# yml-bit/CTA-GAN

Measured on AMD Instinct MI355X. Metric: paired 512x512 slices/sec (G+D step); generator rel-L2 vs CPU reference, higher is better.
Workload: dtype bf16; 1 GPU; HdGan stage-2 full G+D train step (G, Reg, STN, D_m, losses, Adam x3), 16 paired 512x512 slices/GPU; per_gpu_batch=16, global_batch=16, size=512, parallelism=single, rccl_ranks=1, dp_backend=none

## Files before the change

### cta_gan_amd/csrc/common.h

```cpp
#pragma once
#include <hip/hip_runtime.h>
#include <stdint.h>
#include <utility>
#include "../../include/ctagan_hip.h"

#define CTG_OK 0
#define CTG_EINVAL 1

enum { DT_F32 = 0, DT_BF16 = 1, DT_PAIR = 2, DT_MIX = 3 };
enum { ACT_NONE = 0, ACT_RELU = 1, ACT_LRELU = 2, ACT_TANH = 3, ACT_SIGMOID = 4 };
enum { PAD_ZERO = 0, PAD_REFLECT = 1 };

typedef __bf16 bf16_t;
struct bfpair_t { bf16_t v; };
typedef float f32x4 __attribute__((ext_vector_type(4)));
typedef unsigned u32x4 __attribute__((ext_vector_type(4)));
typedef __bf16 bf16x8 __attribute__((ext_vector_type(8)));
typedef __bf16 bf16x4 __attribute__((ext_vector_type(4)));

#define LRELU_SLOPE 0.2f

#define CTG_ENTER() (void)hipGetLastError()

static inline int ctg_launch_status() {
// ... 72 lines not shown
template <> struct Chunk<bfpair_t> {
    static constexpr int N = 8;
    float v[8];
    struct Raw { u32x4 h, l; };
    static __device__ __forceinline__ Raw fetch(const bfpair_t* p, int ld) {
        return Raw{*reinterpret_cast<const u32x4*>(p), *reinterpret_cast<const u32x4*>(p + (ld >> 1))};
    }
    __device__ __forceinline__ void unpack(const Raw& t) {
#pragma unroll
        for (int i = 0; i < 4; ++i) {
            v[2 * i] = __uint_as_float(t.h[i] << 16) + __uint_as_float(t.l[i] << 16);
            v[2 * i + 1] = __uint_as_float(t.h[i] & 0xffff0000u) + __uint_as_float(t.l[i] & 0xffff0000u);
        }
    }
    __device__ __forceinline__ void load(const bfpair_t* p, int ld) { unpack(fetch(p, ld)); }
    __device__ __forceinline__ void store(bfpair_t* p, int ld) const {
        bf16x8 h, l;
#pragma unroll
        for (int i = 0; i < 8; ++i) {
            h[i] = (bf16_t)v[i];
            l[i] = (bf16_t)(v[i] - (float)h[i]);
        }
        *reinterpret_cast<bf16x8*>(p) = h;
        *reinterpret_cast<bf16x8*>(p + (ld >> 1)) = l;
    }
    __device__ __forceinline__ void zero() {
#pragma unroll
        for (int i = 0; i < 8; ++i) v[i] = 0.f;
    }
};
template <typename T> struct PlanesOf { static constexpr int N = 1; };
template <> struct PlanesOf<bfpair_t> { static constexpr int N = 2; };

__device__ __forceinline__ float ld1(const float* p) { return *p; }
__device__ __forceinline__ float ld1(const bf16_t* p) { return (float)*p; }
__device__ __forceinline__ void st1(float* p, float v) { *p = v; }
__device__ __forceinline__ void st1(bf16_t* p, float v) { *p = (bf16_t)v; }

__device__ __forceinline__ float act_apply(float x, int act) {
    switch (act) {
        case ACT_RELU: return x > 0.f ? x : 0.f;
        case ACT_LRELU: return x > 0.f ? x : LRELU_SLOPE * x;
        case ACT_TANH: return tanhf(x);
        case ACT_SIGMOID: return 1.f / (1.f + __expf(-x));
        default: return x;
    }
}
__device__ __forceinline__ float act_grad_from_out(float y, int act) {
    switch (act) {
        case ACT_RELU: return y > 0.f ? 1.f : 0.f;
        case ACT_LRELU: return y > 0.f ? 1.f : LRELU_SLOPE;
        case ACT_TANH: return 1.f - y * y;
        case ACT_SIGMOID: return y * (1.f - y);
        default: return 1.f;
    }
}

template <typename F, int... I>
__device__ __forceinline__ void static_for_impl(F&& f, std::integer_sequence<int, I...>) {
    (f(std::integral_constant<int, I>{}), ...);
}
template <int N, typename F> __device__ __forceinline__ void static_for(F&& f) {
    static_for_impl(static_cast<F&&>(f), std::make_integer_sequence<int, N>{});
}

#define IN_EPS 1e-5f
// ... 36 lines not shown
```

### cta_gan_amd/csrc/conv_wgrad.hip

```cpp
#include <stdlib.h>
#include "conv_dispatch.h"

struct WgradArgs {
    const void* g;
    const void* x;
    float* part;
    int B, Hs, Ws, Mc, g_ld;
    int Hi, Wi, Nc, x_ld;
    int is, pad_mode;
    int slab, sps;
    int ntaps;
    int taps[64];
};

template <typename T> struct WgCfg;
template <> struct WgCfg<bf16_t> { static constexpr int PK = 64, PK_MT = 32, PADB = 32; };
template <> struct WgCfg<float> { static constexpr int PK = 32, PK_MT = 16, PADB = 64; };

template <typename T, int BM, int BN, int NT>
__global__ __launch_bounds__(256) void conv_wgrad_kernel(const WgradArgs a) {
    constexpr int EPC = VecOf<T>::N;
    constexpr int PK = NT > 1 ? WgCfg<T>::PK_MT : WgCfg<T>::PK;
    constexpr int RSM = BM * (int)sizeof(T) + WgCfg<T>::PADB;
    constexpr int RSN = BN * (int)sizeof(T) + WgCfg<T>::PADB;
// ... 919 lines not shown
            const int bm = h.Mc % 64 == 0 ? 64 : h.Mc % 32 == 0 ? 32 : 16, bn = h.Nc % 64 == 0 ? 64 : 32;
            ok = ok && bm >= 32 && !(bm == 32 && bn == 32) && (cnt == 1 || cnt == 2 || cnt == 4) && kw <= 2 && kh <= 2;
            covered += cnt;
            ++nph;
        }
        if (ok && covered == ntaps && ntaps == 9 && nph == 4 && !split) {
            if (taps_3x3(a.taps, false)) {
                WgHaloArgs h = ph[0];
                h.ntaps = 9; h.gtaps = 9; h.kw = 2; h.khb = 2; h.dy0 = -1; h.dx0 = -1; h.py = 0; h.px = 0;
                const int rc = launch_wg_s2m(h, st);
                if (rc != -1) return rc;
            }
        }
        if (ok && covered == ntaps) {
            for (int p = 0; p < nph; ++p) {
                const int rc = launch_wgh_any(ph[p], st);
                if (rc != 0) return rc == -1 ? CTG_EINVAL : rc;
            }
            return split ? 3 : 0;
        }
    }
    if (pair) return 2;
    if (Mc % 32) return CTG_EINVAL;
    return dtype == DT_BF16 ? launch_wg_t<bf16_t>(a, st) : launch_wg_t<float>(a, st);
}

#define RED_MAX_T 24
struct ReduceList {
    const float* part[RED_MAX_T];
    float* dst[RED_MAX_T];
    long sm[RED_MAX_T], sn[RED_MAX_T], stp[RED_MAX_T];
    int Z[RED_MAX_T], ntaps[RED_MAX_T], Mc[RED_MAX_T], Nc[RED_MAX_T], Mreal[RED_MAX_T], Nreal[RED_MAX_T];
    int acc[RED_MAX_T], shift[RED_MAX_T];
    int first[RED_MAX_T + 1];
    int count;
};

__global__ __launch_bounds__(256) void wgrad_reduce_multi_kernel(const ReduceList L) {
    __shared__ float red[256];
    int j = 0;
    while (j + 1 < L.count && (int)blockIdx.x >= L.first[j + 1]) ++j;
    const int shift = L.shift[j], ZP = 1 << shift, IW = 256 >> shift;
    const int il = threadIdx.x & (IW - 1), zq = threadIdx.x >> (8 - shift);
    const int Z = L.Z[j], Mc = L.Mc[j], Nc = L.Nc[j];
    const long E = (long)L.ntaps[j] * Mc * Nc;
    const long idx = (long)((int)blockIdx.x - L.first[j]) * IW + il;
    const float* __restrict__ part = L.part[j];
    float s0 = 0.f, s1 = 0.f, s2 = 0.f, s3 = 0.f;
    if (idx < E) {
        int zz = zq;
        for (; zz + 3 * ZP < Z; zz += 4 * ZP) {
            s0 += part[(long)zz * E + idx];
            s1 += part[(long)(zz + ZP) * E + idx];
            s2 += part[(long)(zz + 2 * ZP) * E + idx];
            s3 += part[(long)(zz + 3 * ZP) * E + idx];
        }
        for (; zz < Z; zz += ZP) s0 += part[(long)zz * E + idx];
    }
    float s = (s0 + s1) + (s2 + s3);
    if (shift) {
        red[zq * IW + il] = s;
        __syncthreads();
        s = 0.f;
        if (zq == 0)
            for (int q = 0; q < ZP; ++q) s += red[q * IW + il];
    }
    if (zq == 0 && idx < E) {
        const int c = (int)(idx % Nc);
        const int m = (int)((idx / Nc) % Mc);
        const int t = (int)(idx / ((long)Nc * Mc));
        if (m < L.Mreal[j] && c < L.Nreal[j]) {
            float* d = L.dst[j] + m * L.sm[j] + c * L.sn[j] + t * L.stp[j];
            *d = L.acc[j] ? *d + s : s;
        }
    }
}

extern "C" int ctg_wgrad_reduce_multi(int count, const void* const* part, void* const* dst, const int* Z,
                                      const int* ntaps, const int* Mc, const int* Nc, const int* Mreal, const int* Nreal,
                                      const long* sm, const long* sn, const long* stp, const int* accumulate,
                                      void* stream) {
    CTG_ENTER();
    if (count < 0) return CTG_EINVAL;
    for (int base = 0; base < count; base += RED_MAX_T) {
        ReduceList L;
        L.count = count - base < RED_MAX_T ? count - base : RED_MAX_T;
        long blocks = 0;
        for (int i = 0; i < L.count; ++i) {
            const int q = base + i;
            if (Z[q] < 1 || ntaps[q] < 1 || Mreal[q] > Mc[q] || Nreal[q] > Nc[q] || part[q] == nullptr || dst[q] == nullptr)
                return CTG_EINVAL;
            const long E = (long)ntaps[q] * Mc[q] * Nc[q];
            const int shift = (Z[q] >= 64 && E <= 65536) ? (E <= 16384 ? 5 : 4) : 0;
            L.part[i] = (const float*)part[q]; L.dst[i] = (float*)dst[q];
            L.sm[i] = sm[q]; L.sn[i] = sn[q]; L.stp[i] = stp[q];
            L.Z[i] = Z[q]; L.ntaps[i] = ntaps[q]; L.Mc[i] = Mc[q]; L.Nc[i] = Nc[q]; L.Mreal[i] = Mreal[q]; L.Nreal[i] = Nreal[q];
            L.acc[i] = accumulate[q]; L.shift[i] = shift;
            L.first[i] = (int)blocks;
            const int iw = 256 >> shift;
            blocks += (E + iw - 1) / iw;
            if (blocks >= (1L << 30)) return CTG_EINVAL;
        }
        L.first[L.count] = (int)blocks;
        if (blocks == 0) continue;
        hipLaunchKernelGGL(wgrad_reduce_multi_kernel, dim3((unsigned)blocks), dim3(256), 0, (hipStream_t)stream, L);
    }
    return ctg_launch_status();
}

extern "C" int ctg_wgrad_reduce(const float* part, int Z, int ntaps, int Mc, int Nc, float* dst, int Mreal, int Nreal,
                                long sm, long sn, long stp, int accumulate, void* stream) {
    CTG_ENTER();
    if (Z < 1 || ntaps < 1 || Mreal > Mc || Nreal > Nc) return CTG_EINVAL;
    const long E = (long)ntaps * Mc * Nc;
    if (Z >= 64 && E <= 65536) {
        if (E <= 16384) {
            hipLaunchKernelGGL(wgrad_reduce_zp_kernel<32>, dim3((unsigned)((E + 7) / 8)), dim3(256), 0,
                               (hipStream_t)stream, part, Z, ntaps, Mc, Nc, dst, Mreal, Nreal, sm, sn, stp, accumulate);
        } else {
            hipLaunchKernelGGL(wgrad_reduce_zp_kernel<16>, dim3((unsigned)((E + 15) / 16)), dim3(256), 0,
                               (hipStream_t)stream, part, Z, ntaps, Mc, Nc, dst, Mreal, Nreal, sm, sn, stp, accumulate);
        }
        return ctg_launch_status();
    }
    const int blocks = (int)((E + 255) / 256 < 4096 ? (E + 255) / 256 : 4096);
    hipLaunchKernelGGL(wgrad_reduce_kernel, dim3(blocks), dim3(256), 0, (hipStream_t)stream, part, Z, ntaps, Mc, Nc,
                       dst, Mreal, Nreal, sm, sn, stp, accumulate);
    return ctg_launch_status();
}
```

### cta_gan_amd/csrc/spatial.hip

```cpp
#include "common.h"

static inline int ew_blocks(long items) {
    long b = (items + 255) / 256;
    return (int)(b < 1 ? 1 : (b > 8192 ? 8192 : b));
}

#define DISPATCH_T(dtype, CALL)                   \
    if ((dtype) == DT_BF16) { typedef bf16_t T; CALL; } \
    else if ((dtype) == DT_F32) { typedef float T; CALL; } \
    else if ((dtype) == DT_PAIR) { typedef bfpair_t T; CALL; } \
    else return CTG_EINVAL;

template <typename T>
__global__ void maxpool2_fwd_kernel(const T* __restrict__ x, int x_ld, T* __restrict__ out, int o_ld, int H, int W,
                                    int C, long items) {
    constexpr int EPC = Chunk<T>::N;
    const int CPP = C / EPC, Ho = H / 2, Wo = W / 2;
    for (long it = (long)blockIdx.x * blockDim.x + threadIdx.x; it < items; it += (long)gridDim.x * blockDim.x) {
        const unsigned pixu = (unsigned)it / (unsigned)CPP;
        const long pix = pixu;
        const int ch = (int)(it - pix * CPP) * EPC;
        const int ox = (int)(pixu % (unsigned)Wo);
        const int oy = (int)((pixu / (unsigned)Wo) % (unsigned)Ho);
        const int n = (int)(pixu / ((unsigned)Wo * (unsigned)Ho));
        const T* base = x + (((size_t)n * H + 2 * oy) * W + 2 * ox) * x_ld + ch;
        Chunk<T> a, b, c, d, o;
        a.load(base, x_ld); b.load(base + x_ld, x_ld); c.load(base + (size_t)W * x_ld, x_ld); d.load(base + (size_t)(W + 1) * x_ld, x_ld);
#pragma unroll
        for (int e = 0; e < EPC; ++e) o.v[e] = fmaxf(fmaxf(a.v[e], b.v[e]), fmaxf(c.v[e], d.v[e]));
        o.store(out + pix * o_ld + ch, o_ld);
    }
}

template <typename T, typename TX = T>
__global__ void maxpool2_bwd_kernel(const TX* __restrict__ x, int x_ld, const T* __restrict__ dout, int d_ld,
                                    T* __restrict__ dx, int dx_ld, int accumulate, int H, int W, int C, long items) {
    constexpr int EPC = Chunk<T>::N;
    const int CPP = C / EPC, Ho = H / 2, Wo = W / 2;
    for (long it = (long)blockIdx.x * blockDim.x + threadIdx.x; it < items; it += (long)gridDim.x * blockDim.x) {
        const unsigned pixu = (unsigned)it / (unsigned)CPP;
        const long pix = pixu;
        const int ch = (int)(it - pix * CPP) * EPC;
        const int xx = (int)(pixu % (unsigned)W);
        const int y = (int)((pixu / (unsigned)W) % (unsigned)H);
        const int n = (int)(pixu / ((unsigned)W * (unsigned)H));
        const int oy = y >> 1, ox = xx >> 1;
        Chunk<T> o;
        o.zero();
        if (oy < Ho && ox < Wo) {
            const TX* base = x + (((size_t)n * H + 2 * oy) * W + 2 * ox) * x_ld + ch;
            Chunk<TX> w[4];
            Chunk<T> g;
            w[0].load(base, x_ld); w[1].load(base + x_ld, x_ld); w[2].load(base + (size_t)W * x_ld, x_ld);
            w[3].load(base + (size_t)(W + 1) * x_ld, x_ld);
            g.load(dout + (((size_t)n * Ho + oy) * Wo + ox) * d_ld + ch, d_ld);
            const int me = (y & 1) * 2 + (xx & 1);
#pragma unroll
            for (int e = 0; e < EPC; ++e) {
                int arg = 0;
                float m = w[0].v[e];
#pragma unroll
                for (int k = 1; k < 4; ++k)
                    if (w[k].v[e] > m) { m = w[k].v[e]; arg = k; }
                o.v[e] = arg == me ? g.v[e] : 0.f;
            }
        }
        T* dst = dx + pix * dx_ld + ch;
        if (accumulate) {
            Chunk<T> prev;
            prev.load(dst, dx_ld);
#pragma unroll
            for (int e = 0; e < EPC; ++e) o.v[e] += prev.v[e];
        }
        o.store(dst, dx_ld);
    }
}

__device__ __forceinline__ void bil_src(int o, float scale, int Hi, int& i0, int& i1, float& l) {
    float s = scale * ((float)o + 0.5f) - 0.5f;
    s = s < 0.f ? 0.f : s;
    i0 = (int)s;
    i1 = i0 + (i0 < Hi - 1 ? 1 : 0);
    l = s - (float)i0;
}

template <typename T>
__global__ void bilinear_fwd_kernel(const T* __restrict__ x, int x_ld, T* __restrict__ out, int o_ld, int Hi, int Wi,
                                    int Ho, int Wo, int C, long items) {
    constexpr int EPC = Chunk<T>::N;
    const int CPP = C / EPC;
    const float sh = (float)Hi / (float)Ho, sw = (float)Wi / (float)Wo;
    for (long it = (long)blockIdx.x * blockDim.x + threadIdx.x; it < items; it += (long)gridDim.x * blockDim.x) {
        const unsigned pixu = (unsigned)it / (unsigned)CPP;
        const long pix = pixu;
        const int ch = (int)(it - pix * CPP) * EPC;
        const int ox = (int)(pixu % (unsigned)Wo);
        const int oy = (int)((pixu / (unsigned)Wo) % (unsigned)Ho);
        const int n = (int)(pixu / ((unsigned)Wo * (unsigned)Ho));
        int y0, y1, x0, x1;
        float ly, lx;
        bil_src(oy, sh, Hi, y0, y1, ly);
        bil_src(ox, sw, Wi, x0, x1, lx);
        const T* b = x + (size_t)n * Hi * Wi * x_ld + ch;
        Chunk<T> v00, v01, v10, v11, o;
        v00.load(b + ((size_t)y0 * Wi + x0) * x_ld, x_ld); v01.load(b + ((size_t)y0 * Wi + x1) * x_ld, x_ld);
        v10.load(b + ((size_t)y1 * Wi + x0) * x_ld, x_ld); v11.load(b + ((size_t)y1 * Wi + x1) * x_ld, x_ld);
        const float hy = 1.f - ly, hx = 1.f - lx;
#pragma unroll
        for (int e = 0; e < EPC; ++e)
            o.v[e] = hy * (hx * v00.v[e] + lx * v01.v[e]) + ly * (hx * v10.v[e] + lx * v11.v[e]);
        o.store(out + pix * o_ld + ch, o_ld);
    }
}

template <typename T>
__global__ void bilinear_bwd_kernel(const T* __restrict__ dout, int d_ld, T* __restrict__ dx, int dx_ld, int Hi,
                                    int Wi, int Ho, int Wo, int C, long items) {
    constexpr int EPC = Chunk<T>::N;
    const int CPP = C / EPC;
    const float sh = (float)Hi / (float)Ho, sw = (float)Wi / (float)Wo;
    for (long it = (long)blockIdx.x * blockDim.x + threadIdx.x; it < items; it += (long)gridDim.x * blockDim.x) {
        const unsigned pixu = (unsigned)it / (unsigned)CPP;
        const long pix = pixu;
        const int ch = (int)(it - pix * CPP) * EPC;
        const int ix = (int)(pixu % (unsigned)Wi);
        const int iy = (int)((pixu / (unsigned)Wi) % (unsigned)Hi);
        const int n = (int)(pixu / ((unsigned)Wi * (unsigned)Hi));
        float wy[5], wx[5];
#pragma unroll
        for (int k = 0; k < 5; ++k) {
            const int oy = 2 * iy - 2 + k, ox = 2 * ix - 2 + k;
            wy[k] = 0.f; wx[k] = 0.f;
            if (oy >= 0 && oy < Ho) {
                int a0, a1; float l;
                bil_src(oy, sh, Hi, a0, a1, l);
                wy[k] = (a0 == iy ? 1.f - l : 0.f) + (a1 == iy ? l : 0.f);
            }
            if (ox >= 0 && ox < Wo) {
                int a0, a1; float l;
                bil_src(ox, sw, Wi, a0, a1, l);
                wx[k] = (a0 == ix ? 1.f - l : 0.f) + (a1 == ix ? l : 0.f);
            }
        }
        Chunk<T> o;
        o.zero();
        const T* b = dout + (size_t)n * Ho * Wo * d_ld + ch;
        for (int a = 0; a < 5; ++a) {
            if (wy[a] == 0.f) continue;
            const int oy = 2 * iy - 2 + a;
            for (int c = 0; c < 5; ++c) {
                if (wx[c] == 0.f) continue;
                const int ox = 2 * ix - 2 + c;
                Chunk<T> g;
                g.load(b + ((size_t)oy * Wo + ox) * d_ld, d_ld);
                const float w = wy[a] * wx[c];
#pragma unroll
                for (int e = 0; e < EPC; ++e) o.v[e] += w * g.v[e];
            }
        }
        o.store(dx + pix * dx_ld + ch, dx_ld);
    }
}

template <typename T>
__global__ void chan_pad_kernel(const float* __restrict__ src, int Cs, T* __restrict__ dst, int Cpad, long P) {
    constexpr int EPC = Chunk<T>::N;
    const int CPP = Cpad / EPC;
    for (long pix = (long)blockIdx.x * blockDim.x + threadIdx.x; pix < P; pix += (long)gridDim.x * blockDim.x) {
        Chunk<T> o;
        o.zero();
        if (Cs == 2 && ((uintptr_t)src & 7) == 0) {
            const float2 v = *reinterpret_cast<const float2*>(src + pix * 2);
            o.v[0] = v.x; o.v[1] = v.y;
        } else {
            for (int c = 0; c < Cs; ++c) o.v[c] = src[pix * Cs + c];
        }
        constexpr int PL = PlanesOf<T>::N;
        T* d = dst + pix * Cpad * PL;
        o.store(d, Cpad * PL);
        o.zero();
        for (int cc = 1; cc < CPP; ++cc) o.store(d + cc * EPC, Cpad * PL);
    }
}

template <typename T>
__global__ void im2col_pack_kernel(const float* __restrict__ s0, const float* __restrict__ s1, int Cin, int Hi, int Wi,
                                   int kh, int kw, int stride, int pad, int pad_mode, T* __restrict__ dst, int Ho,
                                   int Wo, int Kpad, long items) {
    constexpr int EPC = Chunk<T>::N;
    const int CPP = Kpad / EPC;
    const int K = Cin * kh * kw;
    for (long it = (long)blockIdx.x * blockDim.x + threadIdx.x; it < items; it += (long)gridDim.x * blockDim.x) {
        const unsigned pixu = (unsigned)it / (unsigned)CPP;
        const long pix = pixu;
        const int cc = (int)(it - pix * CPP);
        const int ox = (int)(pixu % (unsigned)Wo);
        const int oy = (int)((pixu / (unsigned)Wo) % (unsigned)Ho);
        const int n = (int)(pixu / ((unsigned)Wo * (unsigned)Ho));
        Chunk<T> o;
#pragma unroll
        for (int e = 0; e < EPC; ++e) {
            const int k = cc * EPC + e;
            float v = 0.f;
            if (k < K) {
                const int c = k / (kh * kw);
                const int r = k - c * kh * kw;
                const int ky = r / kw, kx = r - ky * kw;
                int iy = oy * stride - pad + ky, ix = ox * stride - pad + kx;
                bool ok = true;
                if (pad_mode == PAD_REFLECT) { iy = reflect_idx(iy, Hi); ix = reflect_idx(ix, Wi); }
                else ok = (unsigned)iy < (unsigned)Hi && (unsigned)ix < (unsigned)Wi;
                if (ok) v = (c == 0 ? s0 : s1)[((size_t)n * Hi + iy) * Wi + ix];
            }
            o.v[e] = v;
        }
        o.store(dst + pix * Kpad * PlanesOf<T>::N + cc * EPC, Kpad * PlanesOf<T>::N);
    }
}

template <typename T>
__global__ void copy_channels_kernel(const T* __restrict__ src, int s_ld, T* __restrict__ dst, int d_ld, int C,
                                     long items) {
    constexpr int EPC = Chunk<T>::N;
    const int CPP = C / EPC;
    for (long it = (long)blockIdx.x * blockDim.x + threadIdx.x; it < items; it += (long)gridDim.x * blockDim.x) {
        const unsigned pixu = (unsigned)it / (unsigned)CPP;
        const long pix = pixu;
        const int ch = (int)(it - pix * CPP) * EPC;
        *reinterpret_cast<u32x4*>(dst + pix * d_ld + ch) = *reinterpret_cast<const u32x4*>(src + pix * s_ld + ch);
        if constexpr (PlanesOf<T>::N == 2)
            *reinterpret_cast<u32x4*>(dst + pix * d_ld + (d_ld >> 1) + ch) = *reinterpret_cast<const u32x4*>(src + pix * s_ld + (s_ld >> 1) + ch);
    }
}

extern "C" int ctg_maxpool2_fwd(int dtype, const void* x, int x_ld, void* out, int o_ld, int B, int H, int W, int C,
                                void* stream) {
    CTG_ENTER();
    const int epc = dtype == DT_F32 ? 4 : 8;
    if (C % epc || H < 2 || W < 2) return CTG_EINVAL;
    const long items = (long)B * (H / 2) * (W / 2) * (C / epc);
    if (items >= (1L << 31)) return CTG_EINVAL;
    DISPATCH_T(dtype, hipLaunchKernelGGL((maxpool2_fwd_kernel<T>), dim3(ew_blocks(items)), dim3(256), 0,
                                         (hipStream_t)stream, (const T*)x, x_ld, (T*)out, o_ld, H, W, C, items));
    return ctg_launch_status();
}

extern "C" int ctg_maxpool2_bwd(int dtype, const void* x, int x_ld, const void* dout, int d_ld, void* dx, int dx_ld,
                                int accumulate, int B, int H, int W, int C, void* stream) {
    CTG_ENTER();
    const int epc = dtype == DT_F32 ? 4 : 8;
    if (C % epc || H < 2 || W < 2) return CTG_EINVAL;
    const long items = (long)B * H * W * (C / epc);
    if (items >= (1L << 31)) return CTG_EINVAL;
    if (dtype == DT_MIX) {
        hipLaunchKernelGGL((maxpool2_bwd_kernel<bf16_t, bfpair_t>), dim3(ew_blocks(items)), dim3(256), 0, (hipStream_t)stream,
                           (const bfpair_t*)x, x_ld, (const bf16_t*)dout, d_ld, (bf16_t*)dx, dx_ld, accumulate, H, W, C, items);
        return ctg_launch_status();
    }
    DISPATCH_T(dtype, hipLaunchKernelGGL((maxpool2_bwd_kernel<T>), dim3(ew_blocks(items)), dim3(256), 0,
                                         (hipStream_t)stream, (const T*)x, x_ld, (const T*)dout, d_ld, (T*)dx, dx_ld,
                                         accumulate, H, W, C, items));
    return ctg_launch_status();
}

extern "C" int ctg_bilinear_fwd(int dtype, const void* x, int x_ld, void* out, int o_ld, int B, int Hi, int Wi, int Ho,
                                int Wo, int C, void* stream) {
    CTG_ENTER();
    const int epc = dtype == DT_F32 ? 4 : 8;
    if (C % epc) return CTG_EINVAL;
    const long items = (long)B * Ho * Wo * (C / epc);
    if (items >= (1L << 31)) return CTG_EINVAL;
    DISPATCH_T(dtype, hipLaunchKernelGGL((bilinear_fwd_kernel<T>), dim3(ew_blocks(items)), dim3(256), 0,
                                         (hipStream_t)stream, (const T*)x, x_ld, (T*)out, o_ld, Hi, Wi, Ho, Wo, C,
                                         items));
    return ctg_launch_status();
}

extern "C" int ctg_bilinear_bwd(int dtype, const void* dout, int d_ld, void* dx, int dx_ld, int B, int Hi, int Wi,
                                int Ho, int Wo, int C, void* stream) {
    CTG_ENTER();
    const int epc = dtype == DT_F32 ? 4 : 8;
    if (C % epc || Ho != 2 * Hi || Wo != 2 * Wi) return CTG_EINVAL;
    const long items = (long)B * Hi * Wi * (C / epc);
    if (items >= (1L << 31)) return CTG_EINVAL;
    DISPATCH_T(dtype, hipLaunchKernelGGL((bilinear_bwd_kernel<T>), dim3(ew_blocks(items)), dim3(256), 0,
                                         (hipStream_t)stream, (const T*)dout, d_ld, (T*)dx, dx_ld, Hi, Wi, Ho, Wo, C,
                                         items));
    return ctg_launch_status();
}

__global__ void split_weights_kernel(const float* __restrict__ x, long x_ld, bf16_t* __restrict__ out, int C, long P) {
    const int cpp = C / 8;
    const long items = P * cpp;
    for (long it = (long)blockIdx.x * blockDim.x + threadIdx.x; it < items; it += (long)gridDim.x * blockDim.x) {
        const long p = it / cpp;
        const int c = (int)(it - p * cpp) * 8;
        const float* src = x + p * x_ld + c;
        const f32x4 a = *reinterpret_cast<const f32x4*>(src), b = *reinterpret_cast<const f32x4*>(src + 4);
        bf16x8 hi, lo;
#pragma unroll
        for (int e = 0; e < 4; ++e) {
            hi[e] = (bf16_t)a[e];
            lo[e] = (bf16_t)(a[e] - (float)hi[e]);
            hi[4 + e] = (bf16_t)b[e];
            lo[4 + e] = (bf16_t)(b[e] - (float)hi[4 + e]);
        }
        bf16_t* row = out + p * (2L * C);
        const int j = c >> 5, i = c & 31;
        *reinterpret_cast<bf16x8*>(row + 64 * j + i) = hi;
        *reinterpret_cast<bf16x8*>(row + 64 * j + 32 + i) = lo;
    }
}

extern "C" int ctg_split_weights(const float* x, long x_ld, void* out, int C, long P, void* stream) {
    CTG_ENTER();
    if (C < 32 || C % 32 || x_ld < C || x_ld % 4 || P < 1 || ((uintptr_t)x & 15) || ((uintptr_t)out & 15)) return CTG_EINVAL;
    hipLaunchKernelGGL(split_weights_kernel, dim3(ew_blocks(P * (C / 8))), dim3(256), 0, (hipStream_t)stream, x, x_ld,
                       (bf16_t*)out, C, P);
    return ctg_launch_status();
}
// ... 75 lines not shown
    const int cpp = C / 8;
    for (long it = (long)blockIdx.x * blockDim.x + threadIdx.x; it < items; it += (long)gridDim.x * blockDim.x) {
        const long p = it / cpp;
        const int c = (int)(it - p * cpp) * 8;
        Chunk<bfpair_t> v;
        v.load(src + p * s_ld + c, s_ld);
        Chunk<float> a, b;
#pragma unroll
        for (int e = 0; e < 4; ++e) { a.v[e] = v.v[e]; b.v[e] = v.v[4 + e]; }
        a.store(dst + p * d_ld + c);
        b.store(dst + p * d_ld + c + 4);
    }
}

extern "C" int ctg_pair_convert(int dir, const void* src, long s_ld, void* dst, long d_ld, int C, long P, void* stream) {
    CTG_ENTER();
    if (C < 8 || C % 8 || P < 1 || (dir != 0 && dir != 1) || ((uintptr_t)src & 15) || ((uintptr_t)dst & 15)) return CTG_EINVAL;
    const long pl = dir == 0 ? d_ld : s_ld, fl = dir == 0 ? s_ld : d_ld;
    if (pl < 2 * C || pl % 16 || pl >= (1L << 31) || fl < C || fl % 4) return CTG_EINVAL;
    const long items = P * (C / 8);
    if (dir == 0)
        hipLaunchKernelGGL(pair_from_f32_kernel, dim3(ew_blocks(items)), dim3(256), 0, (hipStream_t)stream, (const float*)src,
                           s_ld, (bfpair_t*)dst, (int)d_ld, C, items);
    else
        hipLaunchKernelGGL(pair_to_f32_kernel, dim3(ew_blocks(items)), dim3(256), 0, (hipStream_t)stream,
                           (const bfpair_t*)src, (int)s_ld, (float*)dst, d_ld, C, items);
    return ctg_launch_status();
}

extern "C" int ctg_chan_pad(int dtype, const float* src, int Cs, void* dst, int Cpad, long P, void* stream) {
    CTG_ENTER();
    const int epc = dtype == DT_F32 ? 4 : 8;
    if (Cs < 1 || Cs > 4 || Cpad % epc || P * (Cpad / epc) >= (1L << 31)) return CTG_EINVAL;
    DISPATCH_T(dtype, hipLaunchKernelGGL((chan_pad_kernel<T>), dim3(ew_blocks(P)), dim3(256), 0,
                                         (hipStream_t)stream, src, Cs, (T*)dst, Cpad, P));
    return ctg_launch_status();
}

extern "C" int ctg_im2col_pack(int dtype, const float* s0, const float* s1, int Cin, int B, int Hi, int Wi, int kh,
                               int kw, int stride, int pad, int pad_mode, void* dst, int Ho, int Wo, int Kpad,
                               void* stream) {
    CTG_ENTER();
    const int epc = dtype == DT_F32 ? 4 : 8;
    if (Cin < 1 || Cin > 2 || (Cin == 2 && s1 == nullptr) || Kpad % epc || Kpad < Cin * kh * kw) return CTG_EINVAL;
    if (pad_mode == PAD_REFLECT && (pad >= Hi || pad >= Wi)) return CTG_EINVAL;
    if (Ho != (Hi + 2 * pad - kh) / stride + 1 || Wo != (Wi + 2 * pad - kw) / stride + 1) return CTG_EINVAL;
    const long items = (long)B * Ho * Wo * (Kpad / epc);
    if (items >= (1L << 31)) return CTG_EINVAL;
    DISPATCH_T(dtype, hipLaunchKernelGGL((im2col_pack_kernel<T>), dim3(ew_blocks(items)), dim3(256), 0,
                                         (hipStream_t)stream, s0, s1, Cin, Hi, Wi, kh, kw, stride, pad, pad_mode,
                                         (T*)dst, Ho, Wo, Kpad, items));
    return ctg_launch_status();
}

extern "C" int ctg_copy_channels(int dtype, const void* src, int s_ld, void* dst, int d_ld, int C, long P,
                                 void* stream) {
    CTG_ENTER();
    const int epc = dtype == DT_F32 ? 4 : 8;
    if (C % epc || s_ld % epc || d_ld % epc) return CTG_EINVAL;
    const long items = P * (C / epc);
    if (items >= (1L << 31)) return CTG_EINVAL;
    DISPATCH_T(dtype, hipLaunchKernelGGL((copy_channels_kernel<T>), dim3(ew_blocks(items)), dim3(256), 0,
                                         (hipStream_t)stream, (const T*)src, s_ld, (T*)dst, d_ld, C, items));
    return ctg_launch_status();
}

extern "C" int ctg_abi_version(void) { return CTG_ABI_VERSION; }
```

Baseline: 332.5 slices/s.

## Restructure spatial elementwise kernels around per-output-cell streaming and vectorized wgrad reduce

Maxpool backward now runs one thread per pooled cell that writes all four input pixels, instead of one thread per input pixel that re-reads the whole 2x2 window. Bilinear 2x upsampling forward and backward get dedicated kernels that share neighbour loads across output pixels, driven by a generic issue/finish item-streaming helper. Channel padding is parallelised per chunk rather than per pixel, and the wgrad split-K reduction gains a float4-vectorised path with deeper load batching. These changes aim to cut redundant global loads and index arithmetic in memory-bound kernels, at the cost of more code and per-item register pressure.

```diff
diff --git a/cta_gan_amd/csrc/common.h b/cta_gan_amd/csrc/common.h
--- a/cta_gan_amd/csrc/common.h
+++ b/cta_gan_amd/csrc/common.h
@@ -128,6 +128,65 @@
 template <typename T> struct PlanesOf { static constexpr int N = 1; };
 template <> struct PlanesOf<bfpair_t> { static constexpr int N = 2; };
 
+struct ItemPos { int c, x, y, n; };
+__device__ __forceinline__ ItemPos item_decode(unsigned it, int CPP, int W, int H) {
+    ItemPos p;
+    const unsigned pix = it / (unsigned)CPP, row = pix / (unsigned)W;
+    p.c = (int)(it - pix * (unsigned)CPP);
+    p.x = (int)(pix - row * (unsigned)W);
+    p.n = (int)(row / (unsigned)H);
+    p.y = (int)(row - (unsigned)p.n * (unsigned)H);
+    return p;
+}
+__device__ __forceinline__ void item_advance(ItemPos& p, const ItemPos& d, int CPP, int W, int H) {
+    p.c += d.c;
+    int k = p.c >= CPP ? 1 : 0;
+    p.c -= k ? CPP : 0;
+    p.x += d.x + k;
+    k = p.x >= W ? 1 : 0;
+    p.x -= k ? W : 0;
+    p.y += d.y + k;
+    k = p.y >= H ? 1 : 0;
+    p.y -= k ? H : 0;
+    p.n += d.n + k;
+}
+
+#define STREAM_THREADS 256
+template <int UNR, typename Op>
+__device__ __forceinline__ void stream_items(const Op& op, long items, int CPP, int W, int H) {
+    const long S = (long)gridDim.x * STREAM_THREADS;
+    long it = (long)blockIdx.x * STREAM_THREADS + threadIdx.x;
+    if (it >= items) return;
+    ItemPos p = item_decode((unsigned)it, CPP, W, H);
+    const ItemPos d = item_decode((unsigned)S, CPP, W, H);
+    if constexpr (UNR > 1) {
+        for (; it + (UNR - 1) * S < items; it += UNR * S) {
+            typename Op::Req r[UNR];
+            ItemPos q[UNR];
+#pragma unroll
+            for (int u = 0; u < UNR; ++u) {
+                q[u] = p;
+                op.issue(r[u], p);
+                item_advance(p, d, CPP, W, H);
+            }
+            __builtin_amdgcn_sched_barrier(0);
+#pragma unroll
+            for (int u = 0; u < UNR; ++u) {
+                op.finish(r[u], q[u]);
+                __builtin_amdgcn_sched_barrier(0);
+            }
+        }
+    }
+    for (; it < items; it += S) {
+        typename Op::Req r;
+        op.issue(r, p);
+        __builtin_amdgcn_sched_barrier(0);
+        op.finish(r, p);
+        __builtin_amdgcn_sched_barrier(0);
+        item_advance(p, d, CPP, W, H);
+    }
+}
+
 __device__ __forceinline__ float ld1(const float* p) { return *p; }
 __device__ __forceinline__ float ld1(const bf16_t* p) { return (float)*p; }
 __device__ __forceinline__ void st1(float* p, float v) { *p = v; }
diff --git a/cta_gan_amd/csrc/conv_wgrad.hip b/cta_gan_amd/csrc/conv_wgrad.hip
--- a/cta_gan_amd/csrc/conv_wgrad.hip
+++ b/cta_gan_amd/csrc/conv_wgrad.hip
@@ -975,14 +975,83 @@
     long sm[RED_MAX_T], sn[RED_MAX_T], stp[RED_MAX_T];
     int Z[RED_MAX_T], ntaps[RED_MAX_T], Mc[RED_MAX_T], Nc[RED_MAX_T], Mreal[RED_MAX_T], Nreal[RED_MAX_T];
     int acc[RED_MAX_T], shift[RED_MAX_T];
+    int vec[RED_MAX_T];
     int first[RED_MAX_T + 1];
     int count;
 };
 
+__device__ __forceinline__ void wgrad_reduce_vec4(const ReduceList& L, int j, f32x4* red) {
+    const int shift = L.shift[j], ZP = 1 << shift, IW = 256 >> shift;
+    const int il = threadIdx.x & (IW - 1), zq = threadIdx.x >> (8 - shift);
+    const int Z = L.Z[j], Mc = L.Mc[j], Nc = L.Nc[j];
+    const long E = (long)L.ntaps[j] * Mc * Nc;
+    const long idx = ((long)((int)blockIdx.x - L.first[j]) * IW + il) * 4;
+    f32x4 s0 = {0.f, 0.f, 0.f, 0.f}, s1 = s0, s2 = s0, s3 = s0;
+    if (idx < E) {
+        const float* __restrict__ base = L.part[j] + idx;
+        const long step = (long)ZP * E;
+        long off = (long)zq * E;
+        int zz = zq;
+        for (; zz + 7 * ZP < Z; zz += 8 * ZP) {
+            f32x4 v[8];
+#pragma unroll
+            for (int k = 0; k < 8; ++k) {
+                v[k] = *reinterpret_cast<const f32x4*>(base + off);
+                off += step;
+                asm volatile("" : "+v"(off));
+            }
+            __builtin_amdgcn_sched_barrier(0);
+            s0 += v[0]; s1 += v[1]; s2 += v[2]; s3 += v[3];
+            s0 += v[4]; s1 += v[5]; s2 += v[6]; s3 += v[7];
+        }
+        for (; zz + 3 * ZP < Z; zz += 4 * ZP) {
+            f32x4 v[4];
+#pragma unroll
+            for (int k = 0; k < 4; ++k) v[k] = *reinterpret_cast<const f32x4*>(base + off + k * step);
+            __builtin_amdgcn_sched_barrier(0);
+            s0 += v[0]; s1 += v[1]; s2 += v[2]; s3 += v[3];
+            off += 4 * step;
+        }
+        for (; zz < Z; zz += ZP) {
+            s0 += *reinterpret_cast<const f32x4*>(base + off);
+            off += step;
+        }
+    }
+    f32x4 s = (s0 + s1) + (s2 + s3);
+    if (shift) {
+        red[zq * IW + il] = s;
+        __syncthreads();
+        s = f32x4{0.f, 0.f, 0.f, 0.f};
+        if (zq == 0)
+            for (int q = 0; q < ZP; ++q) s += red[q * IW + il];
+    }
+    if (zq == 0 && idx < E) {
+        int c = (int)(idx % Nc);
+        int m = (int)((idx / Nc) % Mc);
+        int t = (int)(idx / ((long)Nc * Mc));
+#pragma unroll
+        for (int e = 0; e < 4; ++e) {
+            if (m < L.Mreal[j] && c < L.Nreal[j]) {
+                float* d = L.dst[j] + m * L.sm[j] + c * L.sn[j] + t * L.stp[j];
+                *d = L.acc[j] ? *d + s[e] : s[e];
+            }
+            if (++c == Nc) {
+                c = 0;
+                if (++m == Mc) { m = 0; ++t; }
+            }
+        }
+    }
+}
+
 __global__ __launch_bounds__(256) void wgrad_reduce_multi_kernel(const ReduceList L) {
-    __shared__ float red[256];
+    __shared__ f32x4 red4[256];
+    float* red = reinterpret_cast<float*>(red4);
     int j = 0;
     while (j + 1 < L.count && (int)blockIdx.x >= L.first[j + 1]) ++j;
+    if (L.vec[j]) {
+        wgrad_reduce_vec4(L, j, red4);
+        return;
+    }
     const int shift = L.shift[j], ZP = 1 << shift, IW = 256 >> shift;
     const int il = threadIdx.x & (IW - 1), zq = threadIdx.x >> (8 - shift);
     const int Z = L.Z[j], Mc = L.Mc[j], Nc = L.Nc[j];
@@ -1035,12 +1104,13 @@
                 return CTG_EINVAL;
             const long E = (long)ntaps[q] * Mc[q] * Nc[q];
             const int shift = (Z[q] >= 64 && E <= 65536) ? (E <= 16384 ? 5 : 4) : 0;
+            const int vec = (shift > 0 && E % 4 == 0 && ((uintptr_t)part[q] & 15) == 0) ? 1 : 0;
             L.part[i] = (const float*)part[q]; L.dst[i] = (float*)dst[q];
             L.sm[i] = sm[q]; L.sn[i] = sn[q]; L.stp[i] = stp[q];
             L.Z[i] = Z[q]; L.ntaps[i] = ntaps[q]; L.Mc[i] = Mc[q]; L.Nc[i] = Nc[q]; L.Mreal[i] = Mreal[q]; L.Nreal[i] = Nreal[q];
-            L.acc[i] = accumulate[q]; L.shift[i] = shift;
+            L.acc[i] = accumulate[q]; L.shift[i] = shift; L.vec[i] = vec;
             L.first[i] = (int)blocks;
-            const int iw = 256 >> shift;
+            const long iw = (long)(256 >> shift) * (vec ? 4 : 1);
             blocks += (E + iw - 1) / iw;
             if (blocks >= (1L << 30)) return CTG_EINVAL;
         }
diff --git a/cta_gan_amd/csrc/spatial.hip b/cta_gan_amd/csrc/spatial.hip
--- a/cta_gan_amd/csrc/spatial.hip
+++ b/cta_gan_amd/csrc/spatial.hip
@@ -2,6 +2,11 @@
 
 static inline int ew_blocks(long items) {
     long b = (items + 255) / 256;
+    return (int)(b < 1 ? 1 : (b > 8192 ? 8192 : b));
+}
+
+static inline int ew_blocks_unr(long items, int unr) {
+    long b = (items + 256L * unr - 1) / (256L * unr);
     return (int)(b < 1 ? 1 : (b > 8192 ? 8192 : b));
 }
 
@@ -32,48 +37,81 @@
     }
 }
 
-template <typename T, typename TX = T>
-__global__ void maxpool2_bwd_kernel(const TX* __restrict__ x, int x_ld, const T* __restrict__ dout, int d_ld,
-                                    T* __restrict__ dx, int dx_ld, int accumulate, int H, int W, int C, long items) {
-    constexpr int EPC = Chunk<T>::N;
-    const int CPP = C / EPC, Ho = H / 2, Wo = W / 2;
-    for (long it = (long)blockIdx.x * blockDim.x + threadIdx.x; it < items; it += (long)gridDim.x * blockDim.x) {
-        const unsigned pixu = (unsigned)it / (unsigned)CPP;
-        const long pix = pixu;
-        const int ch = (int)(it - pix * CPP) * EPC;
-        const int xx = (int)(pixu % (unsigned)W);
-        const int y = (int)((pixu / (unsigned)W) % (unsigned)H);
-        const int n = (int)(pixu / ((unsigned)W * (unsigned)H));
-        const int oy = y >> 1, ox = xx >> 1;
+template <typename T, typename TX, bool ACC> struct PoolBwdOp {
+    const TX* x; int x_ld; const T* dout; int d_ld; T* dx; int dx_ld; int H, W, Ho, Wo;
+    struct Req { typename Chunk<TX>::Raw w[4]; typename Chunk<T>::Raw g, prev[4]; T* dst; };
+    __device__ __forceinline__ size_t off(int k) const { return (size_t)((k >> 1) * W + (k & 1)) * dx_ld; }
+    __device__ __forceinline__ void issue(Req& r, const ItemPos& p) const {
+        const int ch = p.c * Chunk<T>::N;
+        const size_t pix = ((size_t)p.n * H + 2 * p.y) * W + 2 * p.x;
+        const TX* base = x + pix * x_ld + ch;
+        r.w[0] = Chunk<TX>::fetch(base, x_ld);
+        r.w[1] = Chunk<TX>::fetch(base + x_ld, x_ld);
+        r.w[2] = Chunk<TX>::fetch(base + (size_t)W * x_ld, x_ld);
+        r.w[3] = Chunk<TX>::fetch(base + (size_t)(W + 1) * x_ld, x_ld);
+        r.g = Chunk<T>::fetch(dout + (((size_t)p.n * Ho + p.y) * Wo + p.x) * d_ld + ch, d_ld);
+        r.dst = dx + pix * dx_ld + ch;
+        if constexpr (ACC) {
+#pragma unroll
+            for (int k = 0; k < 4; ++k) r.prev[k] = Chunk<T>::fetch(r.dst + off(k), dx_ld);
+        }
+    }
+    __device__ __forceinline__ void rest_px(T* d) const {
         Chunk<T> o;
         o.zero();
-        if (oy < Ho && ox < Wo) {
-            const TX* base = x + (((size_t)n * H + 2 * oy) * W + 2 * ox) * x_ld + ch;
-            Chunk<TX> w[4];
-            Chunk<T> g;
-            w[0].load(base, x_ld); w[1].load(base + x_ld, x_ld); w[2].load(base + (size_t)W * x_ld, x_ld);
-            w[3].load(base + (size_t)(W + 1) * x_ld, x_ld);
-            g.load(dout + (((size_t)n * Ho + oy) * Wo + ox) * d_ld + ch, d_ld);
-            const int me = (y & 1) * 2 + (xx & 1);
-#pragma unroll
-            for (int e = 0; e < EPC; ++e) {
-                int arg = 0;
-                float m = w[0].v[e];
-#pragma unroll
-                for (int k = 1; k < 4; ++k)
-                    if (w[k].v[e] > m) { m = w[k].v[e]; arg = k; }
-                o.v[e] = arg == me ? g.v[e] : 0.f;
+        if constexpr (ACC) {
+            Chunk<T> prev;
+            prev.load(d, dx_ld);
+#pragma unroll
+            for (int e = 0; e < Chunk<T>::N; ++e) o.v[e] += prev.v[e];
+        }
+        o.store(d, dx_ld);
+    }
+    __device__ __forceinline__ void finish(const Req& r, const ItemPos& p) const {
+        constexpr int EPC = Chunk<T>::N;
+        Chunk<TX> w[4];
+        Chunk<T> g;
+#pragma unroll
+        for (int k = 0; k < 4; ++k) w[k].unpack(r.w[k]);
+        g.unpack(r.g);
+        int arg[EPC];
+#pragma unroll
+        for (int e = 0; e < EPC; ++e) {
+            arg[e] = 0;
+            float m = w[0].v[e];
+#pragma unroll
+            for (int k = 1; k < 4; ++k)
+                if (w[k].v[e] > m) { m = w[k].v[e]; arg[e] = k; }
+        }
+#pragma unroll
+        for (int k = 0; k < 4; ++k) {
+            Chunk<T> o;
+#pragma unroll
+            for (int e = 0; e < EPC; ++e) o.v[e] = arg[e] == k ? g.v[e] : 0.f;
+            if constexpr (ACC) {
+                Chunk<T> prev;
+                prev.unpack(r.prev[k]);
+#pragma unroll
+                for (int e = 0; e < EPC; ++e) o.v[e] += prev.v[e];
             }
-        }
-        T* dst = dx + pix * dx_ld + ch;
-        if (accumulate) {
-            Chunk<T> prev;
-            prev.load(dst, dx_ld);
-#pragma unroll
-            for (int e = 0; e < EPC; ++e) o.v[e] += prev.v[e];
-        }
-        o.store(dst, dx_ld);
-    }
+            o.store(r.dst + off(k), dx_ld);
+        }
+        const bool lastx = (W & 1) && p.x == Wo - 1, lasty = (H & 1) && p.y == Ho - 1;
+        if (lastx) {
+            rest_px(r.dst + (size_t)2 * dx_ld);
+            rest_px(r.dst + (size_t)(W + 2) * dx_ld);
+        }
+        if (lasty) {
+            rest_px(r.dst + (size_t)2 * W * dx_ld);
+            rest_px(r.dst + (size_t)(2 * W + 1) * dx_ld);
+            if (lastx) rest_px(r.dst + (size_t)(2 * W + 2) * dx_ld);
+        }
+    }
+};
+
+template <typename T, typename TX, bool ACC>
+__global__ __launch_bounds__(256) void maxpool2_bwd_kernel(const PoolBwdOp<T, TX, ACC> op, int CPP, long items) {
+    stream_items<1>(op, items, CPP, op.Wo, op.Ho);
 }
 
 __device__ __forceinline__ void bil_src(int o, float scale, int Hi, int& i0, int& i1, float& l) {
@@ -84,12 +122,20 @@
     l = s - (float)i0;
 }
 
+__device__ __forceinline__ void bil_src_ratio(int o, int Hi, int Ho, int& i0, int& i1, float& l) {
+    long num = (long)(2 * o + 1) * Hi - Ho;
+    num = num < 0 ? 0 : num;
+    const long den = 2L * Ho;
+    i0 = (int)(num / den);
+    i1 = i0 + (i0 < Hi - 1 ? 1 : 0);
+    l = (float)(num - i0 * den) / (float)den;
+}
+
 template <typename T>
 __global__ void bilinear_fwd_kernel(const T* __restrict__ x, int x_ld, T* __restrict__ out, int o_ld, int Hi, int Wi,
                                     int Ho, int Wo, int C, long items) {
     constexpr int EPC = Chunk<T>::N;
     const int CPP = C / EPC;
-    const float sh = (float)Hi / (float)Ho, sw = (float)Wi / (float)Wo;
     for (long it = (long)blockIdx.x * blockDim.x + threadIdx.x; it < items; it += (long)gridDim.x * blockDim.x) {
         const unsigned pixu = (unsigned)it / (unsigned)CPP;
         const long pix = pixu;
@@ -99,8 +145,8 @@
         const int n = (int)(pixu / ((unsigned)Wo * (unsigned)Ho));
         int y0, y1, x0, x1;
         float ly, lx;
-        bil_src(oy, sh, Hi, y0, y1, ly);
-        bil_src(ox, sw, Wi, x0, x1, lx);
+        bil_src_ratio(oy, Hi, Ho, y0, y1, ly);
+        bil_src_ratio(ox, Wi, Wo, x0, x1, lx);
         const T* b = x + (size_t)n * Hi * Wi * x_ld + ch;
         Chunk<T> v00, v01, v10, v11, o;
         v00.load(b + ((size_t)y0 * Wi + x0) * x_ld, x_ld); v01.load(b + ((size_t)y0 * Wi + x1) * x_ld, x_ld);
@@ -113,73 +159,183 @@
     }
 }
 
-template <typename T>
-__global__ void bilinear_bwd_kernel(const T* __restrict__ dout, int d_ld, T* __restrict__ dx, int dx_ld, int Hi,
-                                    int Wi, int Ho, int Wo, int C, long items) {
-    constexpr int EPC = Chunk<T>::N;
-    const int CPP = C / EPC;
-    const float sh = (float)Hi / (float)Ho, sw = (float)Wi / (float)Wo;
-    for (long it = (long)blockIdx.x * blockDim.x + threadIdx.x; it < items; it += (long)gridDim.x * blockDim.x) {
-        const unsigned pixu = (unsigned)it / (unsigned)CPP;
-        const long pix = pixu;
-        const int ch = (int)(it - pix * CPP) * EPC;
-        const int ix = (int)(pixu % (unsigned)Wi);
-        const int iy = (int)((pixu / (unsigned)Wi) % (unsigned)Hi);
-        const int n = (int)(pixu / ((unsigned)Wi * (unsigned)Hi));
-        float wy[5], wx[5];
-#pragma unroll
-        for (int k = 0; k < 5; ++k) {
-            const int oy = 2 * iy - 2 + k, ox = 2 * ix - 2 + k;
-            wy[k] = 0.f; wx[k] = 0.f;
-            if (oy >= 0 && oy < Ho) {
-                int a0, a1; float l;
+template <typename T> struct Bil2FwdOp {
+    const T* x; int x_ld; T* out; int o_ld; int Hi, Wi, Ho, Wo;
+    struct Req { typename Chunk<T>::Raw v00, v01, v10, v11; };
+    __device__ __forceinline__ void issue(Req& r, const ItemPos& p) const {
+        const int y0 = p.y > 0 ? p.y - 1 : 0, x0 = p.x > 0 ? p.x - 1 : 0;
+        const int y1 = y0 + (y0 < Hi - 1 ? 1 : 0), x1 = x0 + (x0 < Wi - 1 ? 1 : 0);
+        const T* b = x + (size_t)p.n * Hi * Wi * x_ld + p.c * Chunk<T>::N;
+        r.v00 = Chunk<T>::fetch(b + ((size_t)y0 * Wi + x0) * x_ld, x_ld);
+        r.v01 = Chunk<T>::fetch(b + ((size_t)y0 * Wi + x1) * x_ld, x_ld);
+        r.v10 = Chunk<T>::fetch(b + ((size_t)y1 * Wi + x0) * x_ld, x_ld);
+        r.v11 = Chunk<T>::fetch(b + ((size_t)y1 * Wi + x1) * x_ld, x_ld);
+    }
+    __device__ __forceinline__ void finish(const Req& r, const ItemPos& p) const {
+        constexpr int EPC = Chunk<T>::N;
+        const float sh = (float)Hi / (float)Ho, sw = (float)Wi / (float)Wo;
+        Chunk<T> v00, v01, v10, v11;
+        v00.unpack(r.v00); v01.unpack(r.v01); v10.unpack(r.v10); v11.unpack(r.v11);
+        T* ob = out + (size_t)p.n * Ho * Wo * o_ld + p.c * EPC;
+#pragma unroll
+        for (int jy = 0; jy < 2; ++jy) {
+            const int oy = 2 * p.y - 1 + jy;
+            if (oy < 0 || oy >= Ho) continue;
+            int t0, t1;
+            float ly;
+            bil_src(oy, sh, Hi, t0, t1, ly);
+            const float hy = 1.f - ly;
+#pragma unroll
+            for (int jx = 0; jx < 2; ++jx) {
+                const int ox = 2 * p.x - 1 + jx;
+                if (ox < 0 || ox >= Wo) continue;
+                float lx;
+                bil_src(ox, sw, Wi, t0, t1, lx);
+                const float hx = 1.f - lx;
+                Chunk<T> o;
+                {
+#pragma clang fp contract(off)
+#pragma unroll
+                    for (int e = 0; e < EPC; ++e) {
+                        const float t = __fmaf_rn(hx, v00.v[e], lx * v01.v[e]), u = __fmaf_rn(hx, v10.v[e], lx * v11.v[e]);
+                        o.v[e] = __fmaf_rn(hy, t, ly * u);
+                    }
+                }
+                o.store(ob + ((size_t)oy * Wo + ox) * o_ld, o_ld);
+            }
+        }
+    }
+};
+template <typename T> struct BilUnr { static constexpr int FWD = 2; };
+template <> struct BilUnr<bfpair_t> { static constexpr int FWD = 1; };
+
+template <typename T>
+__global__ __launch_bounds__(256) void bilinear2_fwd_kernel(const Bil2FwdOp<T> op, int CPP, long items) {
+    stream_items<BilUnr<T>::FWD>(op, items, CPP, op.Wi + 1, op.Hi + 1);
+}
+
+template <typename T, int RP> struct Bil2BwdOp {
+    const T* dout; int d_ld; T* dx; int dx_ld; int Hi, Wi, Ho, Wo;
+    struct Req { typename Chunk<T>::Raw g[RP][6]; };
+    __device__ __forceinline__ void fetch_rows(Req& r, const ItemPos& p, int r0) const {
+        const T* b = dout + (size_t)p.n * Ho * Wo * d_ld + p.c * Chunk<T>::N;
+        size_t co[6];
+#pragma unroll
+        for (int q = 0; q < 6; ++q) {
+            int ox = 4 * p.x - 1 + q;
+            ox = ox < 0 ? 0 : (ox > Wo - 1 ? Wo - 1 : ox);
+            co[q] = (size_t)ox * d_ld;
+        }
+#pragma unroll
+        for (int k = 0; k < RP; ++k) {
+            int oy = 4 * p.y - 1 + r0 + k;
+            oy = oy < 0 ? 0 : (oy > Ho - 1 ? Ho - 1 : oy);
+            const T* row = b + (size_t)oy * Wo * d_ld;
+#pragma unroll
+            for (int q = 0; q < 6; ++q) r.g[k][q] = Chunk<T>::fetch(row + co[q], d_ld);
+        }
+    }
+    __device__ __forceinline__ void issue(Req& r, const ItemPos& p) const { fetch_rows(r, p, 0); }
+    __device__ __forceinline__ void finish(Req& r, const ItemPos& p) const {
+        constexpr int EPC = Chunk<T>::N;
+        const float sh = (float)Hi / (float)Ho, sw = (float)Wi / (float)Wo;
+        float wy[2][4], wx[2][4];
+#pragma unroll
+        for (int d = 0; d < 2; ++d) {
+            const int iy = 2 * p.y + d, ix = 2 * p.x + d;
+#pragma unroll
+            for (int k = 0; k < 4; ++k) {
+                const int oy = 2 * iy - 1 + k, ox = 2 * ix - 1 + k;
+                int a0, a1;
+                float l;
                 bil_src(oy, sh, Hi, a0, a1, l);
-                wy[k] = (a0 == iy ? 1.f - l : 0.f) + (a1 == iy ? l : 0.f);
+                wy[d][k] = (oy >= 0 && oy < Ho) ? (a0 == iy ? 1.f - l : 0.f) + (a1 == iy ? l : 0.f) : 0.f;
+                bil_src(ox, sw, Wi, a0, a1, l);
+                wx[d][k] = (ox >= 0 && ox < Wo) ? (a0 == ix ? 1.f - l : 0.f) + (a1 == ix ? l : 0.f) : 0.f;
             }
-            if (ox >= 0 && ox < Wo) {
-                int a0, a1; float l;
-                bil_src(ox, sw, Wi, a0, a1, l);
-                wx[k] = (a0 == ix ? 1.f - l : 0.f) + (a1 == ix ? l : 0.f);
+        }
+        Chunk<T> o[2][2];
+        o[0][0].zero(); o[0][1].zero(); o[1][0].zero(); o[1][1].zero();
+#pragma unroll
+        for (int ph = 0; ph < 6 / RP; ++ph) {
+            if (ph > 0) {
+                __builtin_amdgcn_sched_barrier(0);
+                fetch_rows(r, p, ph * RP);
+                __builtin_amdgcn_sched_barrier(0);
             }
+#pragma unroll
+            for (int k = 0; k < RP; ++k) {
+                const int row = ph * RP + k;
+#pragma unroll
+                for (int q = 0; q < 6; ++q) {
+                    Chunk<T> g;
+                    g.unpack(r.g[k][q]);
+#pragma unroll
+                    for (int dy = 0; dy < 2; ++dy) {
+                        const int a = row - 2 * dy;
+                        if (a < 0 || a > 3) continue;
+#pragma unroll
+                        for (int dxx = 0; dxx < 2; ++dxx) {
+                            const int c = q - 2 * dxx;
+                            if (c < 0 || c > 3) continue;
+                            const bool on = wy[dy][a] != 0.f && wx[dxx][c] != 0.f;
+                            const float w = wy[dy][a] * wx[dxx][c];
+#pragma unroll
+                            for (int e = 0; e < EPC; ++e)
+                                o[dy][dxx].v[e] = on ? __fmaf_rn(w, g.v[e], o[dy][dxx].v[e]) : o[dy][dxx].v[e];
+                        }
+                    }
+                    __builtin_amdgcn_sched_barrier(0);
+                }
+            }
+        }
+        T* d0 = dx + (((size_t)p.n * Hi + 2 * p.y) * Wi + 2 * p.x) * dx_ld + p.c * EPC;
+        const bool y1 = 2 * p.y + 1 < Hi, x1 = 2 * p.x + 1 < Wi;
+        o[0][0].store(d0, dx_ld);
+        if (x1) o[0][1].store(d0 + dx_ld, dx_ld);
+        if (y1) o[1][0].store(d0 + (size_t)Wi * dx_ld, dx_ld);
+        if (y1 && x1) o[1][1].store(d0 + (size_t)(Wi + 1) * dx_ld, dx_ld);
+    }
+};
+template <typename T> struct BilBwdRows { static constexpr int N = 3; };
+template <> struct BilBwdRows<bfpair_t> { static constexpr int N = 2; };
+
+template <typename T>
+__global__ __launch_bounds__(256) void bilinear2_bwd_kernel(const Bil2BwdOp<T, BilBwdRows<T>::N> op, int CPP, long items) {
+    stream_items<1>(op, items, CPP, (op.Wi + 1) / 2, (op.Hi + 1) / 2);
+}
+
+template <typename T>
+__global__ __launch_bounds__(256) void chan_pad_kernel(const float* __restrict__ src, int Cs, T* __restrict__ dst, int Cpad, long items) {
+    constexpr int EPC = Chunk<T>::N, PL = PlanesOf<T>::N;
+    const int CPP = Cpad / EPC;
+    const long S = (long)gridDim.x * 256;
+    long it = (long)blockIdx.x * 256 + threadIdx.x;
+    if (it >= items) return;
+    long pix = (long)((unsigned)it / (unsigned)CPP);
+    int cc = (int)(it - pix * CPP);
+    const long dp = (long)((unsigned)S / (unsigned)CPP);
+    const int dc = (int)(S - dp * CPP);
+    const bool vec2 = Cs == 2 && ((uintptr_t)src & 7) == 0;
+    for (; it < items; it += S) {
+        float v[4] = {0.f, 0.f, 0.f, 0.f};
+        if (vec2) {
+            const float2 t = *reinterpret_cast<const float2*>(src + pix * 2);
+            v[0] = t.x; v[1] = t.y;
+        } else {
+#pragma unroll
+            for (int c = 0; c < 4; ++c)
+                if (c < Cs) v[c] = src[pix * Cs + c];
         }
         Chunk<T> o;
         o.zero();
-        const T* b = dout + (size_t)n * Ho * Wo * d_ld + ch;
-        for (int a = 0; a < 5; ++a) {
-            if (wy[a] == 0.f) continue;
-            const int oy = 2 * iy - 2 + a;
-            for (int c = 0; c < 5; ++c) {
-                if (wx[c] == 0.f) continue;
-                const int ox = 2 * ix - 2 + c;
-                Chunk<T> g;
-                g.load(b + ((size_t)oy * Wo + ox) * d_ld, d_ld);
-                const float w = wy[a] * wx[c];
-#pragma unroll
-                for (int e = 0; e < EPC; ++e) o.v[e] += w * g.v[e];
-            }
-        }
-        o.store(dx + pix * dx_ld + ch, dx_ld);
-    }
-}
-
-template <typename T>
-__global__ void chan_pad_kernel(const float* __restrict__ src, int Cs, T* __restrict__ dst, int Cpad, long P) {
-    constexpr int EPC = Chunk<T>::N;
-    const int CPP = Cpad / EPC;
-    for (long pix = (long)blockIdx.x * blockDim.x + threadIdx.x; pix < P; pix += (long)gridDim.x * blockDim.x) {
-        Chunk<T> o;
-        o.zero();
-        if (Cs == 2 && ((uintptr_t)src & 7) == 0) {
-            const float2 v = *reinterpret_cast<const float2*>(src + pix * 2);
-            o.v[0] = v.x; o.v[1] = v.y;
-        } else {
-            for (int c = 0; c < Cs; ++c) o.v[c] = src[pix * Cs + c];
-        }
-        constexpr int PL = PlanesOf<T>::N;
-        T* d = dst + pix * Cpad * PL;
-        o.store(d, Cpad * PL);
-        o.zero();
-        for (int cc = 1; cc < CPP; ++cc) o.store(d + cc * EPC, Cpad * PL);
+#pragma unroll
+        for (int c = 0; c < 4; ++c) o.v[c] = cc == 0 ? v[c] : 0.f;
+        o.store(dst + pix * Cpad * PL + cc * EPC, Cpad * PL);
+        cc += dc;
+        const int k = cc >= CPP ? 1 : 0;
+        cc -= k ? CPP : 0;
+        pix += dp + k;
     }
 }
 
@@ -245,22 +401,40 @@
     return ctg_launch_status();
 }
 
+template <typename T, typename TX>
+static void launch_pool_bwd(const void* x, int x_ld, const void* dout, int d_ld, void* dx, int dx_ld, int accumulate, int H,
+                            int W, int C, long items, hipStream_t st) {
+    const dim3 grid(ew_blocks(items));
+    const int CPP = C / Chunk<T>::N;
+    if (accumulate) {
+        const PoolBwdOp<T, TX, true> op{(const TX*)x, x_ld, (const T*)dout, d_ld, (T*)dx, dx_ld, H, W, H / 2, W / 2};
+        hipLaunchKernelGGL((maxpool2_bwd_kernel<T, TX, true>), grid, dim3(256), 0, st, op, CPP, items);
+    } else {
+        const PoolBwdOp<T, TX, false> op{(const TX*)x, x_ld, (const T*)dout, d_ld, (T*)dx, dx_ld, H, W, H / 2, W / 2};
+        hipLaunchKernelGGL((maxpool2_bwd_kernel<T, TX, false>), grid, dim3(256), 0, st, op, CPP, items);
+    }
+}
+
 extern "C" int ctg_maxpool2_bwd(int dtype, const void* x, int x_ld, const void* dout, int d_ld, void* dx, int dx_ld,
                                 int accumulate, int B, int H, int W, int C, void* stream) {
     CTG_ENTER();
     const int epc = dtype == DT_F32 ? 4 : 8;
     if (C % epc || H < 2 || W < 2) return CTG_EINVAL;
-    const long items = (long)B * H * W * (C / epc);
-    if (items >= (1L << 31)) return CTG_EINVAL;
+    if ((long)B * H * W * (C / epc) >= (1L << 31)) return CTG_EINVAL;
+    const long items = (long)B * (H / 2) * (W / 2) * (C / epc);
     if (dtype == DT_MIX) {
-        hipLaunchKernelGGL((maxpool2_bwd_kernel<bf16_t, bfpair_t>), dim3(ew_blocks(items)), dim3(256), 0, (hipStream_t)stream,
-                           (const bfpair_t*)x, x_ld, (const bf16_t*)dout, d_ld, (bf16_t*)dx, dx_ld, accumulate, H, W, C, items);
+        launch_pool_bwd<bf16_t, bfpair_t>(x, x_ld, dout, d_ld, dx, dx_ld, accumulate, H, W, C, items, (hipStream_t)stream);
         return ctg_launch_status();
     }
-    DISPATCH_T(dtype, hipLaunchKernelGGL((maxpool2_bwd_kernel<T>), dim3(ew_blocks(items)), dim3(256), 0,
-                                         (hipStream_t)stream, (const T*)x, x_ld, (const T*)dout, d_ld, (T*)dx, dx_ld,
-                                         accumulate, H, W, C, items));
-    return ctg_launch_status();
+    DISPATCH_T(dtype, (launch_pool_bwd<T, T>(x, x_ld, dout, d_ld, dx, dx_ld, accumulate, H, W, C, items, (hipStream_t)stream)));
+    return ctg_launch_status();
+}
+
+template <typename T>
+static void launch_bil2_fwd(const void* x, int x_ld, void* out, int o_ld, int Hi, int Wi, int C, long cells, hipStream_t st) {
+    const Bil2FwdOp<T> op{(const T*)x, x_ld, (T*)out, o_ld, Hi, Wi, 2 * Hi, 2 * Wi};
+    hipLaunchKernelGGL((bilinear2_fwd_kernel<T>), dim3(ew_blocks_unr(cells, BilUnr<T>::FWD)), dim3(256), 0, st, op,
+                       C / Chunk<T>::N, cells);
 }
 
 extern "C" int ctg_bilinear_fwd(int dtype, const void* x, int x_ld, void* out, int o_ld, int B, int Hi, int Wi, int Ho,
@@ -270,10 +444,25 @@
     if (C % epc) return CTG_EINVAL;
     const long items = (long)B * Ho * Wo * (C / epc);
     if (items >= (1L << 31)) return CTG_EINVAL;
+    if (Ho == 2 * Hi && Wo == 2 * Wi && Hi >= 1 && Wi >= 1) {
+        const long cells = (long)B * (Hi + 1) * (Wi + 1) * (C / epc);
+        if (cells < (1L << 31)) {
+            DISPATCH_T(dtype, launch_bil2_fwd<T>(x, x_ld, out, o_ld, Hi, Wi, C, cells, (hipStream_t)stream));
+            return ctg_launch_status();
+        }
+    }
     DISPATCH_T(dtype, hipLaunchKernelGGL((bilinear_fwd_kernel<T>), dim3(ew_blocks(items)), dim3(256), 0,
                                          (hipStream_t)stream, (const T*)x, x_ld, (T*)out, o_ld, Hi, Wi, Ho, Wo, C,
                                          items));
     return ctg_launch_status();
+}
+
+template <typename T>
+static void launch_bil2_bwd(const void* dout, int d_ld, void* dx, int dx_ld, int B, int Hi, int Wi, int C, hipStream_t st) {
+    const Bil2BwdOp<T, BilBwdRows<T>::N> op{(const T*)dout, d_ld, (T*)dx, dx_ld, Hi, Wi, 2 * Hi, 2 * Wi};
+    const int CPP = C / Chunk<T>::N;
+    const long items = (long)B * ((Hi + 1) / 2) * ((Wi + 1) / 2) * CPP;
+    hipLaunchKernelGGL((bilinear2_bwd_kernel<T>), dim3(ew_blocks(items)), dim3(256), 0, st, op, CPP, items);
 }
 
 extern "C" int ctg_bilinear_bwd(int dtype, const void* dout, int d_ld, void* dx, int dx_ld, int B, int Hi, int Wi,
@@ -283,9 +472,7 @@
     if (C % epc || Ho != 2 * Hi || Wo != 2 * Wi) return CTG_EINVAL;
     const long items = (long)B * Hi * Wi * (C / epc);
     if (items >= (1L << 31)) return CTG_EINVAL;
-    DISPATCH_T(dtype, hipLaunchKernelGGL((bilinear_bwd_kernel<T>), dim3(ew_blocks(items)), dim3(256), 0,
-                                         (hipStream_t)stream, (const T*)dout, d_ld, (T*)dx, dx_ld, Hi, Wi, Ho, Wo, C,
-                                         items));
+    DISPATCH_T(dtype, launch_bil2_bwd<T>(dout, d_ld, dx, dx_ld, B, Hi, Wi, C, (hipStream_t)stream));
     return ctg_launch_status();
 }
 
@@ -427,8 +614,9 @@
     CTG_ENTER();
     const int epc = dtype == DT_F32 ? 4 : 8;
     if (Cs < 1 || Cs > 4 || Cpad % epc || P * (Cpad / epc) >= (1L << 31)) return CTG_EINVAL;
-    DISPATCH_T(dtype, hipLaunchKernelGGL((chan_pad_kernel<T>), dim3(ew_blocks(P)), dim3(256), 0,
-                                         (hipStream_t)stream, src, Cs, (T*)dst, Cpad, P));
+    const long items = P * (Cpad / epc);
+    DISPATCH_T(dtype, hipLaunchKernelGGL((chan_pad_kernel<T>), dim3(ew_blocks(items)), dim3(256), 0,
+                                         (hipStream_t)stream, src, Cs, (T*)dst, Cpad, items));
     return ctg_launch_status();
 }
 
```

Result: no change. 335.4 slices/s (median of 6 runs) (+0.9%).
